# IllyaArtemchuk/Harmonies-Alphazero

Measured on AMD Instinct MI355X. Metric: self-play env-steps/sec + games/sec @4096 boards, 1/2/4/8 GPUs; bit-exact vs CPU, higher is better.
Workload: dtype u64; 1 GPU; config2: 4096 concurrent boards/GPU, reset + rule-driven play to game end (legal mask, step, chance draws, final scoring); one step = 256 hz_play launches of 4096 boards; boards_per_gpu=4096, parallelism=shard1

## Files before the change

### __graft_entry__.py

```python
import os
import subprocess
import sys

ROOT = os.path.dirname(os.path.abspath(__file__))
PKG = os.path.join(ROOT, "harmonies-alphazero_amd")


def _paths():
    for p in (ROOT, PKG):
        if p not in sys.path:
            sys.path.insert(0, p)


def build() -> None:
    jobs = str(min(16, os.cpu_count() or 4))
    subprocess.run(["make", "-s", "-j", jobs, "-C", PKG], check=True)
    subprocess.run(["make", "-s", "-C", os.path.join(ROOT, "oracle")], check=True)
    _paths()
    import hzamd
    import hzamd._native as nat
    missing = [s for s in nat.exported_symbols() if not hasattr(nat.lib(), s)]
    if missing:
        raise RuntimeError(f"libhz.so lacks symbols: {missing}")


def smoke() -> None:
    _paths()
    import numpy as np
    import torch

    import oracle
    from hzamd.env import BatchedEnv
    from hzamd.state import unpack_ref

    n, base = 256, 4242
    env = BatchedEnv(n, seed_base=base, device="cuda:0")
    env.reset()
    games, steps, _ = env.rollout(max_plies=200)
    st = env.export_state().cpu().numpy()
    torch.cuda.synchronize()
    total, finals, plies, _ = oracle.play_rule_games(n, base)
    got = np.stack([unpack_ref(st[:, b]) for b in range(n)])
    assert (got == finals).all(), "final states differ from the oracle"
    assert (steps.cpu().numpy() == plies).all(), "ply counts differ from the oracle"
    assert int(games.sum()) == n
    for _ in range(15):
        games, steps, _ = env.rollout(max_plies=200, reset=True)
    st = env.export_state().cpu().numpy()
    torch.cuda.synchronize()
    env.check_errors()
    _, finals, plies, _ = oracle.play_rule_games(n, base, episode=15)
    got = np.stack([unpack_ref(st[:, b]) for b in range(n)])
    assert (got == finals).all(), "hz_play: final states differ from the oracle"
    assert (steps.cpu().numpy() == plies).all(), "hz_play: ply counts differ from the oracle"
    env.close()
    print(f"smoke ok: {n} boards, {total} env steps bit-exact vs oracle; hz_play episode 15 bit-exact")


if __name__ == "__main__":
    build()
    if len(sys.argv) > 1 and sys.argv[1] == "smoke":
        smoke()
```

### harmonies-alphazero_amd/csrc/hz_env.hip

```cpp
#include <hip/hip_runtime.h>

#include <cstdio>
#include <cstdlib>
#include <cstring>

#include "../../include/hz_abi.h"
#include "hz_device.hpp"
#include "hz_encode.hpp"
#include "hz_host.hpp"

using namespace hz;
using namespace hz_host;

struct P2Draw {
  int32_t *tag;
  int32_t *k;
  uint64_t *q;
  uint64_t *bag;
  int32_t *c;
};
struct P2Mid {
  int32_t *tag;
  uint64_t *st;
  uint64_t *q;
  int32_t *i;
};

#ifndef HZ_P2_NDRAW
#define HZ_P2_NDRAW 5
#endif
#ifndef HZ_P2_NPLAY
#define HZ_P2_NPLAY 5
#endif
constexpr int kP2Draw = HZ_P2_NDRAW;
constexpr int kP2Play = HZ_P2_NPLAY;
constexpr int kP2SDraw = 4;
constexpr int kP2SPlay = kP2SDraw + kP2Draw;
constexpr int kP2Stages = kP2SPlay + kP2Play;
constexpr int kP2Last = kP2Stages - 1;
constexpr int kP2Ring = kP2Play + 1;
constexpr int kP2Stream = kP2Stages;
static_assert(kP2Draw >= 2 && kP2Draw <= 5 && kP2Play >= 2 && kP2Play <= 5, "stage counts");

struct hz_env {
  DevBufs bufs, p2_bufs, ar_bufs;
  int32_t n;
  uint64_t seed_base;
  hipStream_t stream;
  uint64_t *state;
  uint32_t *mt;
  int32_t *pos;
  int32_t *ply;
  int32_t *episode;
  uint64_t *seed;
  int seed_ahead;
  uint32_t *ahead_mt[2];
  int32_t *ahead_tag[2];
  uint64_t *ahead_pile[2];
  int32_t *ahead_cur[2];
  uint32_t *ahead_rule[2];
  int32_t *ep_final[2];
  size_t nrow;
  uint32_t *ring_mt[3];
  int32_t *ring_tag[3];
  uint64_t *ring_pile[3];
  int32_t *ring_cur[3];
  int32_t *ring_k1[3];
  int calls;
  int primed, slot_valid[2];
  int32_t *mt_src;
  int lazy;
  int ar_ahead;
  uint32_t *ar_mt;
  int32_t *ar_tag;
  uint64_t *ar_pile;
  int32_t *ar_cur;
  int32_t *ar_ep[2];
  int ar_calls, ar_primed;
  uint32_t *pw_words;
  int32_t *pw_tag;
  int32_t *pw_ep;
  uint32_t mt_epoch;
  int pipeline;
  int calls2, primed2;
  int p2_cut[kP2Play - 1];
  int p2_dcut[kP2Draw + 1];
  uint32_t *p2_s[kP2Stream];
  int32_t *p2_s_tag[kP2Stream];
  int32_t *p2_s_cur[kP2Stream];
  uint32_t *p2_p1h[2];
  int32_t *p2_p1t[2];
  uint32_t *p2_p2h[2];
  uint32_t *p2_p3h[2];
  P2Draw p2_x[kP2Draw - 1][2];
  P2Draw p2_pl[kP2Ring];
  P2Mid p2_m[kP2Play - 1][2];
  uint32_t *p2_h[kP2Ring];
  int32_t *p2_h_tag[kP2Ring];
  int32_t *p2_ep[2];
  int32_t *wait_err_own;
  int32_t *wait_err;
  int spin_limit;
};

#ifdef HZ_DIAG
__device__ uint64_t *g_stamps;
__device__ int g_role_only = -1;
#define HZ_STAMP(slot)                                                    \
  do {                                                                    \
    __builtin_amdgcn_sched_barrier(0);                                    \
    if (g_stamps) g_stamps[(size_t)b * 16 + (slot)] = __builtin_amdgcn_s_memtime(); \
    __builtin_amdgcn_sched_barrier(0);                                    \
  } while (0)
#ifndef HZ_DIAG_ROLES_ONLY
#define HZ_ACC(slot, t0)                                                  \
  do {                                                                    \
    __builtin_amdgcn_sched_barrier(0);                                    \
    uint64_t _t = __builtin_amdgcn_s_memtime();                           \
    acc##slot += _t - (t0);                                               \
    t0 = _t;                                                              \
    __builtin_amdgcn_sched_barrier(0);                                    \
  } while (0)
#else
#define HZ_ACC(slot, t0) \
  do {                   \
  } while (0)
#endif
#define HZ_PHASE(slot, t0, b)                                                                 \
  do {                                                                                        \
    __builtin_amdgcn_sched_barrier(0);                                                        \
    if (g_stamps) g_stamps[(size_t)(b) * 16 + (slot)] = __builtin_amdgcn_s_memtime() - (t0); \
    __builtin_amdgcn_sched_barrier(0);                                                        \
  } while (0)
#else
#define HZ_STAMP(slot) \
  do {                 \
  } while (0)
#define HZ_PHASE(slot, t0, b) \
  do {                        \
  } while (0)
#define HZ_ACC(slot, t0) \
  do {                   \
  } while (0)
#endif

namespace {

constexpr int kBlock = 64;

inline int grid_for(int n) { return (n + kBlock - 1) / kBlock; }

constexpr int kStageThreads = 256;
constexpr size_t kResetLds = (size_t)kMT * kLdsStride * sizeof(uint32_t);

__device__ __forceinline__ void stage_mt(uint32_t *__restrict__ g, int nb, int tid, uint64_t mask, bool to_lds) {
  uint32_t *lds = hz_lds;
  constexpr int U = 8;
  int total4 = nb * (kMT / 4);
  for (int q0 = 0; q0 < total4; q0 += kStageThreads * U) {
    uint4 v[U];
#pragma unroll
    for (int u = 0; u < U; u++) {
      int q = q0 + u * kStageThreads + tid;
      int o = q * 4, bl = o / kMT, i = o - bl * kMT;
      if (q < total4 && ((mask >> bl) & 1)) {
        if (to_lds) {
          v[u] = reinterpret_cast<const uint4 *>(g)[q];
        } else {
          v[u].x = lds[i * kLdsStride + bl];
          v[u].y = lds[(i + 1) * kLdsStride + bl];
          v[u].z = lds[(i + 2) * kLdsStride + bl];
          v[u].w = lds[(i + 3) * kLdsStride + bl];
        }
      }
    }
#pragma unroll
    for (int u = 0; u < U; u++) {
      int q = q0 + u * kStageThreads + tid;
      int o = q * 4, bl = o / kMT, i = o - bl * kMT;
      if (q < total4 && ((mask >> bl) & 1)) {
        if (to_lds) {
// ... 1036 lines not shown
            steps += done;
            i += done - 1;
            if (phase_of(s.misc) == PH_OVER) games++;
            continue;
          }
        }
        int a;
        HZ_ACC(8, t0);
        if constexpr (Record) {
          uint64_t mk[3];
          int L = legal_mask(s, mk);
          HZ_ACC(9, t0);
          if (traj_state) {
            uint64_t *o = traj_state + (size_t)i * 6 * n + b;
            o[0] = s.pl[0]; o[(size_t)n] = s.pl[1]; o[(size_t)2 * n] = s.pl[2]; o[(size_t)3 * n] = s.pl[3];
            o[(size_t)4 * n] = s.piles; o[(size_t)5 * n] = s.misc;
          }
          if (traj_mask) {
            uint64_t *o = traj_mask + ((size_t)i * n + b) * 3;
            o[0] = mk[0]; o[1] = mk[1]; o[2] = mk[2];
          }
          a = L ? kth_action(mk, rule_pick_k(rkey, g_ply, L)) : -1;
          if (traj_action) traj_action[(size_t)i * n + b] = (int16_t)a;
        } else {
          a = rule_action(s, rule_h32(rkey, g_ply));
          HZ_ACC(9, t0);
        }
        if (a < 0) break;
        HZ_ACC(10, t0);
        bool te = phase_of(s.misc) == PH_P3;
        step_trusted<true>(s, a, draw);
        if (te) HZ_ACC(12, t0);
        else HZ_ACC(11, t0);
        g_ply++;
        steps++;
        if (phase_of(s.misc) == PH_OVER) games++;
      }
    }
#ifdef HZ_DIAG_ROLES_ONLY
    HZ_PHASE(9, role_t0, b);
#endif
    if (score_pending(s.misc)) finish_game(s);
#ifdef HZ_DIAG_ROLES_ONLY
    HZ_PHASE(10, role_t0, b);
#endif
    HZ_ACC(13, t0);
    store_state(st, n, b, s);
    if (lds_used) pos[b] = draw.m.cursor();
    else if (draw.fell) pos[b] = draw.gm.cursor();
    else pos[b] = cur_b[(size_t)draw.d * n];
    mt_src[b] = lds_used ? -1 : src_b;
    ply[b] = g_ply;
    seed[b] = sd;
#if defined(HZ_DIAG) && !defined(HZ_DIAG_ROLES_ONLY)
    if (g_stamps) {
      uint64_t *o = g_stamps + (size_t)b * 16;
      o[8] = acc8; o[9] = acc9; o[10] = acc10; o[11] = acc11; o[12] = acc12; o[13] = acc13;
    }
#endif
    if (games_done) games_done[b] = games;
    if (steps_done) steps_done[b] = steps;
    if (ep_final) ep_final[b] = episode[b];
    uint64_t lm = __ballot(lds_used);
    if (lane == 0) s_lds_mask = lm;
  }
  if (w0 && !act && lane == 0 && actmask == 0) s_lds_mask = 0;
  __syncthreads();
  uint64_t lds_mask = s_lds_mask & actmask;
  if (lds_mask) stage_mt(g, nb, tid, lds_mask, false);
#ifdef HZ_DIAG
  if (g_stamps && threadIdx.x < 64 && act) g_stamps[(size_t)b * 16 + 5] = __builtin_amdgcn_s_memtime() - role_t0;
#endif
}

#ifndef HZ_P2_ST_WT
#define HZ_P2_ST_WT 0
#endif
#ifndef HZ_P2_AUX
#define HZ_P2_AUX 16
#endif
constexpr int kP2Win = 96;
constexpr int kP2WinRows = kP2Win + 24;
#ifndef HZ_P2_DCUT
#if HZ_P2_NDRAW == 5
#define HZ_P2_DCUT 0, 6, 11, 15, 19
#elif HZ_P2_NDRAW == 4
#define HZ_P2_DCUT 0, 7, 13, 18
#endif
#endif
constexpr int kP2DCut[kP2Draw] = {HZ_P2_DCUT};
constexpr int kP2StageDraws = 7;
#ifndef HZ_P2_PCUT
#if HZ_P2_NPLAY == 5
#define HZ_P2_PCUT 16, 32, 48, 64
#elif HZ_P2_NPLAY == 4
#define HZ_P2_PCUT 24, 40, 56
#endif
#endif
constexpr int kP2PCut[kP2Play - 1] = {HZ_P2_PCUT};
enum { kWvP1 = 8, kWvHash = 9, kWvPlay = 10, kWvIdle = 15 };
#ifndef HZ_P2_WAVES
#if HZ_P2_NDRAW == 5 && HZ_P2_NPLAY == 5
#define HZ_P2_WAVES 0, 1, 4, 9, 2, 3, 8, 10
#elif HZ_P2_NDRAW == 5
#define HZ_P2_WAVES 0, 1, 4, 9, 2, 3, 8, 15
#elif HZ_P2_NPLAY == 5
#define HZ_P2_WAVES 0, 1, 8, 9, 2, 3, 10, 15
#else
#define HZ_P2_WAVES 0, 1, 8, 9, 2, 3, 15, 15
#endif
#endif
constexpr int kP2Wave[8] = {HZ_P2_WAVES};
constexpr int p2_wave_count(int code) {
  int c = 0;
  for (int k = 0; k < 8; k++) c += kP2Wave[k] == code;
  return c;
}
constexpr bool p2_waves_ok() {
  for (int d = 0; d < 5; d++)
    if (p2_wave_count(d) != (d < kP2Draw ? 1 : 0)) return false;
  return p2_wave_count(kWvP1) == 1 && p2_wave_count(kWvHash) == 1 && p2_wave_count(kWvPlay) == (kP2Play == 5 ? 1 : 0);
}
static_assert(p2_waves_ok(), "HZ_P2_WAVES: every stage outside the seed and play blocks on exactly one wave");
constexpr int kP2MinPlies = 96;
#ifdef HZ_DIAG
constexpr int kP2Stamps = 48;
#define P2_PHASE(slot, t0)                                                                                       \
  do {                                                                                                           \
    __builtin_amdgcn_sched_barrier(0);                                                                           \
    if (g_stamps && b < a.n) g_stamps[(size_t)b * kP2Stamps + (slot)] = __builtin_amdgcn_s_memtime() - (t0); \
    __builtin_amdgcn_sched_barrier(0);                                                                           \
  } while (0)
#else
#define P2_PHASE(slot, t0) \
  do {                     \
  } while (0)
#endif
static_assert(4 * kP2WinRows * kWinStride * 4 <= (int)kResetLds, "a window per wave of a draw block");

struct P2Args {
  uint64_t *st;
  uint32_t *mt;
  int32_t *pos, *ply, *episode;
  uint64_t *seed;
  int n, max_plies, draws;
  int cut[kP2Play - 1];
  int dcut[kP2Draw + 1];
  uint64_t seed_base;
  long nrow;
  int32_t *games_done, *steps_done, *mt_src;
  const int32_t *ep_in;
  int32_t *ep_out;
  uint32_t *s_mt[kP2Stages];
  int32_t *s_tag[kP2Stages];
  int32_t *s_cur[kP2Stages];
  int s_idx_last;
  uint32_t *p1h_w;
  const uint32_t *p1h_r;
  int32_t *p1t_w;
  const int32_t *p1t_r;
  uint32_t *p2h_w;
  const uint32_t *p2h_r;
  uint32_t *p3h_w;
  const uint32_t *p3h_r;
  P2Draw x_w[kP2Draw - 1], x_r[kP2Draw - 1];
  P2Draw pl_w, pl_r[kP2Play];
  P2Mid m_w[kP2Play - 1], m_r[kP2Play - 1];
  uint32_t *h_w;
  const uint32_t *h_r[kP2Play];
  int32_t *ht_w;
  const int32_t *ht_r[kP2Play];
  int32_t *err;
  int spin;
};

struct PlayDraw2 {
  uint64_t q0, q1, q2, q3;
  int d, nd;
  bool fell;
  MTR gm;
  const int32_t *cur_nd;
  __device__ __forceinline__ uint32_t pop() {
    uint32_t p9 = (uint32_t)q0 & 0x1FFu;
    q0 = (q0 >> 9) | (q1 << 55);
    q1 = (q1 >> 9) | (q2 << 55);
    q2 = (q2 >> 9) | (q3 << 55);
    q3 >>= 9;
    d++;
    return p9;
  }
  __device__ __forceinline__ bool pair_pops() const { return d + 2 <= nd; }
  __device__ __forceinline__ uint32_t draw_one(uint64_t misc) {
    if (d < nd) return pop();
    if (!fell) {
      gm = MTR(gm.w, gm.stride, *cur_nd);
      fell = true;
    }
    uint32_t p9;
    return draw_pile(misc, gm, p9) ? p9 : 0x1FFu;
  }
  __device__ __forceinline__ uint32_t operator()(uint64_t misc) { return take(misc, true); }
  __device__ __forceinline__ uint32_t take(uint64_t misc, bool want) {
    if (__all(!want || d < nd)) {
      uint32_t p9 = want ? (uint32_t)q0 & 0x1FFu : 0x1FFu;
      uint64_t n0 = (q0 >> 9) | (q1 << 55), n1 = (q1 >> 9) | (q2 << 55), n2 = (q2 >> 9) | (q3 << 55);
      q0 = want ? n0 : q0;
      q1 = want ? n1 : q1;
      q2 = want ? n2 : q2;
      q3 = want ? q3 >> 9 : q3;
      d += want ? 1 : 0;
      return p9;
    }
    return want ? draw_one(misc) : 0x1FFu;
  }
  __device__ __forceinline__ void scripted_reset(State &s) {
    s.pl[0] = s.pl[1] = s.pl[2] = s.pl[3] = 0;
    uint64_t open = q0 & ((1ull << 45) - 1);
    s.piles = open | (5ull << 45);
    uint64_t misc = 0x1FF;
#pragma unroll
    for (int t = 0; t < 6; t++) misc = set_bits(misc, 11 + 5 * t, 5, (uint64_t)initial_count(t));
#pragma unroll
    for (int i = 0; i < 5; i++) apply_pile_fast(misc, (uint32_t)(open >> (9 * i)) & 0x1FFu);
    s.misc = misc;
    q0 = (q0 >> 45) | (q1 << 19);
    q1 = (q1 >> 45) | (q2 << 19);
    q2 = (q2 >> 45) | (q3 << 19);
    q3 >>= 45;
    d = 5;
  }
};

template <class Draw>
__device__ __forceinline__ int p2_plies(State &s, Draw &draw, int g, int g_end, uint64_t rkey, const uint32_t *hs,
                                        size_t nr) {
  const int g0 = g;
  auto hash = [&](int ply) -> uint32_t { return hs && ply < kRulePlies ? hs[(size_t)ply * nr] : rule_h32(rkey, ply); };
  const bool all_hs = __all(hs != nullptr);
  uint32_t hn[8];
  int hn_g = -1;
  while (g < g_end) {
    if (phase_of(s.misc) == PH_OVER) break;
    if (__all(g + 8 <= g_end && turn_pair_safe(s))) {
      uint32_t h[8];
      if (__all(hn_g == g)) {
#pragma unroll
        for (int j = 0; j < 8; j++) h[j] = hn[j];
      } else if (all_hs && __all(g + 8 <= kRulePlies)) {
#pragma unroll
        for (int j = 0; j < 8; j++) h[j] = hs[(size_t)(g + j) * nr];
      } else {
#pragma unroll
        for (int j = 0; j < 8; j++) h[j] = hash(g + j);
      }
// ... 371 lines not shown
__device__ __forceinline__ void p2_draw_stage(const P2Args &a, int b0, int lane, int stage, int base) {
  const int b = b0 + lane;
#ifdef HZ_DIAG
  const uint64_t t0 = __builtin_amdgcn_s_memtime();
#endif
  const bool act = b < a.n;
  const size_t nr = (size_t)a.nrow;
  const int d0 = a.dcut[stage], d1 = stage == kP2Draw - 1 ? a.draws : min(a.draws, a.dcut[stage + 1]);
  const int e = act ? a.ep_in[b] + kP2Last - kP2SDraw - stage : 0;
  const uint32_t *slot = a.s_mt[kP2SDraw + stage];
  int32_t *cur = a.s_cur[kP2SDraw + stage] + b;
  const P2Draw &in = a.x_r[stage > 0 ? stage - 1 : 0];
  const P2Draw &out = stage == kP2Draw - 1 ? a.pl_w : a.x_w[stage < kP2Draw - 1 ? stage : 0];
  bool ok = act && a.s_tag[kP2SDraw + stage][b] == e * 8 + 5;
  int k0 = 0, c0 = kMTAhead;
  uint64_t bag = initial_bag(), q[kAheadWords] = {0, 0, 0, 0};
  constexpr int U = kP2Win / 4;
  const int c4 = (lane & 15) * 4;
  uint4 v[U];
  auto win_load = [&](int r0) {
#pragma unroll
    for (int u = 0; u < U; u++) {
      const int r = r0 + 4 * u + (lane >> 4);
      v[u] = p2_ld4(slot + (size_t)r * nr + b0 + c4);
    }
  };
  auto win_store = [&]() {
#pragma unroll
    for (int u = 0; u < U; u++)
      *reinterpret_cast<uint4 *>(hz_lds + base + (4 * u + (lane >> 4)) * kWinStride + c4) = v[u];
  };
  if (stage == 0) win_load(0);
  if (stage > 0 && act) {
    const int itag = in.tag[b];
    k0 = in.k[b];
    c0 = in.c[b];
    bag = in.bag[b];
#pragma unroll
    for (int i = 0; i < kAheadWords; i++) q[i] = in.q[(size_t)i * nr + b];
    ok = ok && itag == e * 8 + stage;
  }
  const bool draws = ok && k0 >= d0 && d0 < d1;
  const int r0 = wave_min_i(draws ? (c0 & 0xFFFF) : kAheadTwist) & ~3;
  if (r0 < kAheadTwist) {
    if (stage > 0) win_load(r0);
    win_store();
  }
  P2_PHASE(28 + stage, t0);
  if (!act) return;
  if (!ok) {
    out.tag[b] = -1;
    return;
  }
  if (stage == 0) cur[0] = kMTAhead;
  int k = k0, cc = c0;
  if (draws) {
    const int lim = min(r0 + kP2Win, kAheadTwist);
    StreamDraw<WinMT> d{WinMT(base - r0 * kWinStride + lane, c0, lim)};
#pragma unroll 1
    for (int i = d0; i < d1; i++) {
      if (d.m.pos >= lim) break;
      const uint32_t p9 = d(bag);
      if (d.m.pos > lim) break;
      apply_pile_fast(bag, p9);
      const int bit = 9 * i, wd = bit >> 6, off = bit & 63;
      const uint64_t lo9 = (uint64_t)p9 << off, hi9 = off > 55 ? (uint64_t)p9 >> (64 - off) : 0ull;
      q[0] |= wd == 0 ? lo9 : 0ull;
      q[1] |= wd == 1 ? lo9 : wd == 0 ? hi9 : 0ull;
      q[2] |= wd == 2 ? lo9 : wd == 1 ? hi9 : 0ull;
      q[3] |= wd == 3 ? lo9 : wd == 2 ? hi9 : 0ull;
      cc = d.m.cursor();
      p2_st(&cur[(size_t)(i + 1) * nr], cc);
      k = i + 1;
    }
  }
  p2_st(&out.k[b], k);
  p2_st(&out.c[b], cc);
  p2_st(&out.bag[b], bag);
#pragma unroll
  for (int i = 0; i < kAheadWords; i++) p2_st(&out.q[(size_t)i * nr + b], q[i]);
  p2_st(&out.tag[b], e * 8 + stage + 1);
}

__device__ __forceinline__ void p2_hashes(const P2Args &a, int b) {
  const size_t nr = (size_t)a.nrow;
  const int e = a.ep_in[b] + kP2Last - (kP2SPlay - 1);
  const uint64_t rk = rule_key(episode_seed(a.seed_base, b, e));
#pragma unroll 1
  for (int j = 0; j < kRulePlies; j++) p2_st(&a.h_w[(size_t)j * nr + b], rule_h32(rk, j));
  a.ht_w[b] = e;
}

__device__ __forceinline__ void p2_draw(const P2Args &a, int blk, int code) {
  const int tid = threadIdx.x, lane = tid & 63, w = tid >> 6;
  const int b0 = blk * kBlock;
  if (code < kP2Draw) {
    p2_draw_stage(a, b0, lane, code, w * kP2WinRows * kWinStride);
  } else if (code == kWvP1 && b0 + lane < a.n) {
    p2_p1(a, b0 + lane);
  } else if (code == kWvHash && b0 + lane < a.n) {
    p2_hashes(a, b0 + lane);
  }
}

__device__ __forceinline__ void p2_mid_put(const P2Mid &m, size_t nr, int b, const State &s, const PlayDraw2 &d, int g,
                                           int e) {
#pragma unroll
  for (int k = 0; k < 4; k++) p2_st(&m.st[(size_t)k * nr + b], s.pl[k]);
  p2_st(&m.st[4 * nr + b], s.piles);
  p2_st(&m.st[5 * nr + b], s.misc);
  p2_st(&m.q[b], d.q0);
  p2_st(&m.q[nr + b], d.q1);
  p2_st(&m.q[2 * nr + b], d.q2);
  p2_st(&m.q[3 * nr + b], d.q3);
  p2_st(&m.i[b], d.d);
  p2_st(&m.i[nr + b], g);
  p2_st(&m.i[2 * nr + b], d.fell ? d.gm.cursor() : -1);
  p2_st(&m.tag[b], e);
}
__device__ __forceinline__ PlayDraw2 p2_mid_get(const P2Mid &m, size_t nr, int b, State &s, int &g, int nd,
                                               uint32_t *slot, const int32_t *cur) {
#pragma unroll
  for (int k = 0; k < 4; k++) s.pl[k] = m.st[(size_t)k * nr + b];
  s.piles = m.st[4 * nr + b];
  s.misc = m.st[5 * nr + b];
  const int d = m.i[b], fc = m.i[2 * nr + b];
  g = m.i[nr + b];
  return PlayDraw2{m.q[b], m.q[nr + b], m.q[2 * nr + b], m.q[3 * nr + b], d, nd, fc >= 0,
                   MTR(slot, (int)nr, fc >= 0 ? fc : 0), cur + (size_t)nd * nr};
}

__device__ __forceinline__ void p2_play(const P2Args &a, int blk, int st, bool in_block) {
  __shared__ uint64_t s_lds_mask;
  const int tid = threadIdx.x, lane = tid & 63, w = tid >> 6;
  const int b0 = blk * kBlock, b = b0 + lane;
  const bool act = b < a.n;
  const uint64_t actmask = __ballot(act);
  const int nb = a.n - b0 < kBlock ? a.n - b0 : kBlock;
  const size_t nr = (size_t)a.nrow;
#ifdef HZ_DIAG
  const uint64_t t0 = __builtin_amdgcn_s_memtime();
#endif
  const bool last = st == kP2Play - 1;
  bool lds_used = false;
  if (act) {
    const int e = last ? a.episode[b] : a.ep_in[b] + kP2Play - 1 - st;
    const P2Draw &pl = a.pl_r[st];
    const uint32_t *hsrc = a.h_r[st];
    const int32_t *htag = a.ht_r[st];
    uint32_t *slot = a.s_mt[kP2SPlay + st] + b;
    const int32_t *cur = a.s_cur[kP2SPlay + st] + b;
    const int g_end = last ? a.max_plies : min(a.cut[st < kP2Play - 1 ? st : 0], a.max_plies);
    const uint64_t sd = episode_seed(a.seed_base, b, e), rk = rule_key(sd);
    const int ptag = pl.tag[b], nd = pl.k[b];
    const int mtag = st > 0 ? a.m_r[st - 1].tag[b] : e;
    const uint32_t *hs = htag[b] == e ? hsrc + b : nullptr;
    State s;
    int g = 0;
    PlayDraw2 draw = st == 0 ? PlayDraw2{pl.q[b], pl.q[nr + b], pl.q[2 * nr + b], pl.q[3 * nr + b], 0, nd, false,
                                         MTR(slot, (int)nr, 0), cur + (size_t)nd * nr}
                             : p2_mid_get(a.m_r[st - 1], nr, b, s, g, nd, slot, cur);
    const bool prep = ptag == e * 8 + kP2Draw && mtag == e;
    if (prep) {
      if (st == 0) {
        if (__all(nd >= 5)) draw.scripted_reset(s);
        else reset_state(s, draw);
      }
      P2_PHASE(16 + 2 * st, t0);
      g += p2_plies(s, draw, g, g_end, rk, hs, nr);
      P2_PHASE(17 + 2 * st, t0);
    }
    if (!last) {
      const P2Mid &mo = a.m_w[st < kP2Play - 1 ? st : 0];
      if (prep) p2_mid_put(mo, nr, b, s, draw, g, e);
      else mo.tag[b] = -1;
    } else {
      int cursor, src;
      if (prep) {
        cursor = draw.fell ? draw.gm.cursor() : cur[(size_t)draw.d * nr];
        src = 2 + a.s_idx_last;
      } else {
        mt_seed(hz_lds + lane, kLdsStride, sd);
        PlayDraw fb{LdsMT(lane, kMTSeeded), false, false, 0, 0, 0, 0, 0, 0, MT(nullptr, 0), nullptr};
        reset_state(s, fb);
        g = p2_plies(s, fb, 0, a.max_plies, rk, nullptr, nr);
        cursor = fb.m.cursor();
        src = -1;
        lds_used = true;
      }
      a.episode[b] = e + 1;
      if (score_pending(s.misc)) finish_game(s);
      P2_PHASE(27, t0);
      store_state(a.st, a.n, b, s);
      a.pos[b] = cursor;
      a.mt_src[b] = src;
      a.ply[b] = g;
      a.seed[b] = sd;
      a.ep_out[b] = e + 1;
      if (a.games_done) a.games_done[b] = phase_of(s.misc) == PH_OVER ? 1 : 0;
      if (a.steps_done) a.steps_done[b] = g;
    }
#ifdef HZ_DIAG
    if (g_stamps && in_block) g_stamps[(size_t)b * kP2Stamps + w] = __builtin_amdgcn_s_memtime() - t0;
#endif
  }
  if (!in_block) return;
  if (w == 0) {
    const uint64_t lm = __ballot(lds_used);
    if (lane == 0) s_lds_mask = lm;
  }
  __syncthreads();
  const uint64_t lds_mask = s_lds_mask & actmask;
  if (lds_mask) stage_mt(a.mt + (size_t)b0 * kMT, nb, tid, lds_mask, false);
}

__global__ void __launch_bounds__(kStageThreads) __attribute__((amdgpu_waves_per_eu(1, 1))) k_play2(P2Args a, int nblk) {
  const int blk = (int)blockIdx.x;
  const int role = blk / nblk;
  const int rb = blk - role * nblk;
  const int wv = __builtin_amdgcn_readfirstlane((int)(threadIdx.x >> 6));
  const int code = role == 1 || role == 2 ? kP2Wave[4 * (role - 1) + wv] : kWvIdle;
  const int st = role == 0 ? kP2Play - 1 - wv : code == kWvPlay ? 0 : -1;
#ifdef HZ_DIAG
  if (g_role_only >= 0 && g_role_only != role) return;
  const uint64_t t0 = __builtin_amdgcn_s_memtime(), r0 = __builtin_amdgcn_s_memrealtime();
#endif
  if (st >= 0) p2_play(a, rb, st, role == 0);
  else if (role == 3) p2_seed(a, rb);
  else if (role != 0) p2_draw(a, rb, code);
#ifdef HZ_DIAG
  {
    const int w = threadIdx.x >> 6, bb = rb * kBlock + (threadIdx.x & 63);
    const bool idle = (role == 1 || role == 2) && code == kWvIdle;
    if (g_stamps && role > 0 && !idle && bb < a.n) g_stamps[(size_t)bb * kP2Stamps + 4 * role + w] = __builtin_amdgcn_s_memtime() - t0;
    if (g_stamps && bb < a.n && (threadIdx.x & 63) < 4) {
      const int k = threadIdx.x & 63;
      const uint64_t v = k == 0 ? r0 : k == 1 ? __builtin_amdgcn_s_memrealtime() : k == 2 ? t0 : __builtin_amdgcn_s_memtime();
      g_stamps[(size_t)(rb * kBlock + 16 * role + 4 * w + k) * kP2Stamps + 40] = v;
      if (k == 0)
        g_stamps[(size_t)(rb * kBlock + 16 * role + 4 * w) * kP2Stamps + 41] =
            (uint64_t)__builtin_amdgcn_s_getreg((31 << 11) | 4) | ((uint64_t)__builtin_amdgcn_s_getreg((15 << 11) | 20) << 32);
    }
  }
#endif
}
// ... 71 lines not shown
  int b = blockIdx.x * blockDim.x + threadIdx.x;
  if (b >= n) return;
  MT m(mt + (size_t)b * kMT, pos[b]);
  m.normalize();
  pos[b] = m.cursor();
  if (index) index[b] = m.pos;
}

__global__ void __launch_bounds__(kBlock) k_mt_import(int32_t *__restrict__ pos, int n,
                                                      const int32_t *__restrict__ index) {
  int b = blockIdx.x * blockDim.x + threadIdx.x;
  if (b >= n) return;
  pos[b] = index[b] | (kMT << 16);
}

}

__global__ void __launch_bounds__(64) k_mt_materialize(uint32_t *__restrict__ mt, const uint32_t *__restrict__ a0,
                                                      const uint32_t *__restrict__ a1, int32_t *__restrict__ mt_src,
                                                      int n) {
  const int b = blockIdx.x, lane = threadIdx.x;
  const int src = mt_src[b];
  if (src < 0 || src > 1) return;
  const uint32_t *from = (src ? a1 : a0) + (size_t)b * kMT;
  uint32_t *to = mt + (size_t)b * kMT;
  uint32_t v[(kMT + 63) / 64];
#pragma unroll
  for (int k = 0; k < (kMT + 63) / 64; k++) v[k] = lane + 64 * k < kMT ? from[lane + 64 * k] : 0u;
#pragma unroll
  for (int k = 0; k < (kMT + 63) / 64; k++)
    if (lane + 64 * k < kMT) to[lane + 64 * k] = v[k];
  if (lane == 0) mt_src[b] = -1;
}

__global__ void __launch_bounds__(64) k_mt_materialize_ar(uint32_t *__restrict__ mt, const uint32_t *__restrict__ ar_mt,
                                                         int32_t *__restrict__ mt_src, int n) {
  const int b = blockIdx.x, lane = threadIdx.x;
  const int src = mt_src[b];
  if (src < kArSrc || src >= kArSrc + kArSlots) return;
  const uint32_t *from = ar_mt + ((size_t)(src - kArSrc) * n + b) * kMT;
  uint32_t *to = mt + (size_t)b * kMT;
  uint32_t v[(kMT + 63) / 64];
#pragma unroll
  for (int k = 0; k < (kMT + 63) / 64; k++) v[k] = lane + 64 * k < kMT ? from[lane + 64 * k] : 0u;
#pragma unroll
  for (int k = 0; k < (kMT + 63) / 64; k++)
    if (lane + 64 * k < kMT) to[lane + 64 * k] = v[k];
  if (lane == 0) mt_src[b] = -1;
}

static PlyWin ply_win(hz_env *e) {
  return PlyWin{e->pw_words, e->pw_tag, e->pw_ep, (long)e->nrow, (int32_t)e->mt_epoch};
}

static int materialize(hz_env *e) {
  if (!e->lazy) return 0;
  streams_touched(e);
  if (e->ar_mt)
    hipLaunchKernelGGL(k_mt_materialize_ar, dim3(e->n), dim3(64), 0, e->stream, e->mt, e->ar_mt, e->mt_src, e->n);
  hipLaunchKernelGGL(k_mt_materialize, dim3(e->n), dim3(64), 0, e->stream, e->mt, e->ahead_mt[0], e->ahead_mt[1],
                     e->mt_src, e->n);
  if (e->p2_s[0]) {
    P2Slots sl;
    for (int k = 0; k < kP2Stream; k++) sl.s[k] = e->p2_s[k];
    hipLaunchKernelGGL(k_mt_materialize2, dim3(e->n), dim3(64), 0, e->stream, e->mt, sl, e->mt_src,
                       (long)e->nrow);
  }
  e->lazy = 0;
  return launch_err();
}

static_assert(sizeof(((hz_env *)0)->p2_s) / sizeof(uint32_t *) == kP2Stream, "slot ring");

static int p2_clear_tags(hz_env *e) {
  const size_t bytes = e->nrow * sizeof(int32_t);
  auto c = [&](int32_t *t) { return hipMemsetAsync(t, 0xff, bytes, e->stream) != hipSuccess; };
  for (int k = 0; k < kP2Stream; k++)
    if (c(e->p2_s_tag[k])) return 1;
  for (int k = 0; k < 2; k++)
    if (c(e->p2_p1t[k])) return 1;
  for (int k = 0; k < kP2Draw - 1; k++)
    if (c(e->p2_x[k][0].tag) || c(e->p2_x[k][1].tag)) return 1;
  for (int k = 0; k < kP2Ring; k++)
    if (c(e->p2_pl[k].tag) || c(e->p2_h_tag[k])) return 1;
  for (int k = 0; k < kP2Play - 1; k++)
    if (c(e->p2_m[k][0].tag) || c(e->p2_m[k][1].tag)) return 1;
  return 0;
}

static int alloc_p2(hz_env *e) {
  if (e->p2_s[0]) return 0;
  const size_t nr = e->nrow;
  DevBufs &o = e->p2_bufs;
  for (int k = 0; k < kP2Stream; k++) {
    o.get(e->p2_s[k], nr * kMT * 4);
    o.get(e->p2_s_tag[k], nr * 4);
    o.get(e->p2_s_cur[k], (kAheadDraws + 1) * nr * 4);
  }
  auto md = [&](P2Draw &d) {
    o.get(d.tag, nr * 4);
    o.get(d.k, nr * 4);
    o.get(d.q, kAheadWords * nr * 8);
    o.get(d.bag, nr * 8);
    o.get(d.c, nr * 4);
  };
  for (int k = 0; k < kP2Draw - 1; k++) md(e->p2_x[k][0]), md(e->p2_x[k][1]);
  for (int k = 0; k < kP2Ring; k++) {
    md(e->p2_pl[k]);
    o.get(e->p2_h[k], kRulePlies * nr * 4);
    o.get(e->p2_h_tag[k], nr * 4);
  }
  for (int k = 0; k < kP2Play - 1; k++)
    for (int j = 0; j < 2; j++) {
      P2Mid &mm = e->p2_m[k][j];
      o.get(mm.tag, nr * 4);
      o.get(mm.st, 6 * nr * 8);
      o.get(mm.q, 4 * nr * 8);
      o.get(mm.i, 3 * nr * 4);
    }
  for (int k = 0; k < 2; k++) {
    o.get(e->p2_p1h[k], nr * 4);
    o.get(e->p2_p1t[k], nr * 4);
    o.get(e->p2_p2h[k], 4 * nr * 4);
    o.get(e->p2_p3h[k], 4 * nr * 4);
    o.get(e->p2_ep[k], nr * 4);
  }
  if (!o.ok || p2_clear_tags(e)) {
    o.release();
    return 1;
  }
  e->primed2 = 0;
  return 0;
}

static int launch_play2(hz_env *e, int32_t max_plies, int32_t *games_done, int32_t *steps_done) {
  streams_touched(e);
  if (alloc_p2(e)) return 1;
  const int c = e->calls2, r = c & 1, w = r ^ 1;
  if (!e->primed2) {
    if (hipMemcpyAsync(e->p2_ep[w], e->episode, (size_t)e->n * sizeof(int32_t), hipMemcpyDeviceToDevice,
                       e->stream))
      return 1;
    e->primed2 = 1;
  }
  P2Args a{};
  a.st = e->state;
  a.mt = e->mt;
  a.pos = e->pos;
  a.ply = e->ply;
  a.episode = e->episode;
  a.seed = e->seed;
  a.n = e->n;
  a.max_plies = max_plies;
  a.draws = e->seed_ahead;
  a.err = e->wait_err;
  a.spin = e->spin_limit;
  for (int k = 0; k < kP2Play - 1; k++) a.cut[k] = e->p2_cut[k];
  for (int k = 0; k <= kP2Draw; k++) a.dcut[k] = e->p2_dcut[k];
  a.seed_base = e->seed_base;
  a.nrow = (long)e->nrow;
  a.games_done = games_done;
  a.steps_done = steps_done;
  a.mt_src = e->mt_src;
  a.ep_in = e->p2_ep[w];
  a.ep_out = e->p2_ep[r];
  auto sl = [c](int s) { return ((c - s) % kP2Stream + kP2Stream) % kP2Stream; };
  for (int s = 1; s < kP2Stages; s++) {
    a.s_mt[s] = e->p2_s[sl(s)];
    a.s_tag[s] = e->p2_s_tag[sl(s)];
    a.s_cur[s] = e->p2_s_cur[sl(s)];
  }
  a.s_idx_last = sl(kP2Last);
  a.p1h_w = e->p2_p1h[r];
  a.p1h_r = e->p2_p1h[w];
  a.p1t_w = e->p2_p1t[r];
  a.p1t_r = e->p2_p1t[w];
  a.p2h_w = e->p2_p2h[r];
  a.p2h_r = e->p2_p2h[w];
  a.p3h_w = e->p2_p3h[r];
  a.p3h_r = e->p2_p3h[w];
  for (int k = 0; k < kP2Draw - 1; k++) {
    a.x_w[k] = e->p2_x[k][r];
    a.x_r[k] = e->p2_x[k][w];
  }
  a.pl_w = e->p2_pl[c % kP2Ring];
  a.h_w = e->p2_h[c % kP2Ring];
  a.ht_w = e->p2_h_tag[c % kP2Ring];
  for (int st = 0; st < kP2Play; st++) {
    const int k = (c + kP2Ring - 1 - st) % kP2Ring;
    a.pl_r[st] = e->p2_pl[k];
    a.h_r[st] = e->p2_h[k];
    a.ht_r[st] = e->p2_h_tag[k];
  }
  for (int st = 0; st < kP2Play - 1; st++) {
    a.m_w[st] = e->p2_m[st][r];
    a.m_r[st] = e->p2_m[st][w];
  }
  const int nblk = grid_for(e->n);
  hipLaunchKernelGGL(k_play2, dim3(4 * nblk), dim3(kStageThreads), kResetLds, e->stream, a, nblk);
  if (int err = launch_err()) return err;
  e->lazy = 1;
  e->calls2 = (c + 1) % (kP2Stream * kP2Ring * 2);
  e->primed = 0;
  e->ar_primed = 0;
  return 0;
}

extern "C" {

hz_env *hz_env_create(int32_t n_boards, uint64_t seed_base, void *stream) {
  if (n_boards <= 0) return nullptr;
  if (install_comp_table()) return nullptr;
  if (lds_opt_in<k_reset>(kResetLds) || lds_opt_in<k_rollout<false, false>>(kResetLds) ||
      lds_opt_in<k_rollout<false, true>>(kResetLds) || lds_opt_in<k_rollout<true, false>>(kResetLds) ||
      lds_opt_in<k_rollout<true, true>>(kResetLds) || lds_opt_in<k_play2>(kResetLds))
    return nullptr;
  hz_env *e = new (std::nothrow) hz_env();
  if (!e) return nullptr;
  e->n = n_boards;
  e->seed_base = seed_base;
  e->stream = (hipStream_t)stream;
  const size_t n = (size_t)n_boards, nr = (n + kBlock - 1) / kBlock * kBlock, i32 = sizeof(int32_t);
  e->nrow = nr;
  DevBufs &o = e->bufs;
  o.get(e->state, n * 6 * sizeof(uint64_t), 0);
  o.get(e->mt, n * 624 * sizeof(uint32_t));
  o.get(e->pos, n * i32, 0);
  o.get(e->ply, n * i32, 0);
  o.get(e->episode, n * i32, 0);
  o.get(e->seed, n * sizeof(uint64_t), 0);
  o.get(e->mt_src, n * i32, 0xff);
  for (int k = 0; k < 2; k++) {
    o.get(e->ahead_mt[k], n * kMT * sizeof(uint32_t));
    o.get(e->ahead_tag[k], n * i32, 0xff);
    o.get(e->ahead_pile[k], n * kAheadWords * sizeof(uint64_t));
    o.get(e->ahead_cur[k], n * (kAheadDraws + 1) * i32);
    o.get(e->ahead_rule[k], nr * kRulePlies * sizeof(uint32_t));
    o.get(e->ep_final[k], n * i32);
  }
  for (int k = 0; k < kRing; k++) {
    o.get(e->ring_mt[k], nr * kMT * sizeof(uint32_t));
    o.get(e->ring_tag[k], nr * i32, 0xff);
    o.get(e->ring_pile[k], nr * 3 * sizeof(uint64_t));
    o.get(e->ring_cur[k], nr * (kD1Draws + 1) * i32);
    o.get(e->ring_k1[k], nr * i32);
  }
  o.get(e->pw_words, nr * kPlyWin * sizeof(uint32_t));
  o.get(e->pw_tag, nr * i32, 0xff);
  o.get(e->pw_ep, nr * i32, 0);
  o.get(e->wait_err_own, i32, 0);
  e->seed_ahead = kAheadDraws;
  e->ar_ahead = env_pick("HZ_AR_AHEAD", 0, 1);
  e->pipeline = env_pick("HZ_PIPELINE", 1, 2);
  for (int k = 0; k < kP2Play - 1; k++) e->p2_cut[k] = kP2PCut[k];
  if constexpr (kP2Play == 4) env_cuts("HZ_P2_CUTS", e->p2_cut);
  else if constexpr (kP2Play == 5) env_cuts_n("HZ_P2_CUTS5", e->p2_cut, kP2Play - 1, 4, 1 << 20);
  for (int k = 0; k < kP2Draw; k++) e->p2_dcut[k] = kP2DCut[k];
  e->p2_dcut[kP2Draw] = kAheadDraws;
  if constexpr (kP2Draw == 5) {
    int dc[kP2Draw + 1];
    for (int k = 0; k <= kP2Draw; k++) dc[k] = e->p2_dcut[k];
    if (env_cuts_n("HZ_P2_DCUTS", dc + 1, kP2Draw - 1, 1, kAheadDraws - 1) &&
        cuts_gaps_within(dc, kP2Draw + 1, kP2StageDraws))
      for (int k = 0; k <= kP2Draw; k++) e->p2_dcut[k] = dc[k];
  }
  e->mt_epoch = 1;
  e->wait_err = e->wait_err_own;
  e->spin_limit = kSpinLimitDefault;
  if (!o.ok || hipDeviceSynchronize() != hipSuccess) {
    hz_env_destroy(e);
    return nullptr;
  }
  return e;
}

void hz_env_destroy(hz_env *e) {
  if (!e) return;
  e->p2_bufs.release();
  e->ar_bufs.release();
  e->bufs.release();
  delete e;
}

int32_t hz_env_size(const hz_env *e) { return e ? e->n : -1; }

int hz_env_set_error_word(hz_env *e, int32_t *word) {
  if (!e) return -1;
  e->wait_err = word ? word : e->wait_err_own;
  return 0;
}

int hz_env_set_spin_limit(hz_env *e, int32_t limit) {
  if (!e || limit < 0) return -1;
  e->spin_limit = limit ? limit : kSpinLimitDefault;
  return 0;
}

int hz_env_set_pipeline(hz_env *e, int32_t pipeline) {
  if (!e || (pipeline != 1 && pipeline != 2)) return -1;
  e->pipeline = pipeline;
  e->primed = 0;
  e->primed2 = 0;
  return 0;
}

int hz_env_set_auto_ahead(hz_env *e, int32_t on) {
  if (!e) return -1;
  e->ar_ahead = on ? 1 : 0;
  e->ar_primed = 0;
  return 0;
}

int hz_env_set_stream(hz_env *e, void *stream) {
  if (!e) return -1;
  e->stream = (hipStream_t)stream;
  return 0;
}

uint64_t *hz_env_state_ptr(hz_env *e) { return e ? e->state : nullptr; }
uint32_t *hz_env_mt_ptr(hz_env *e) {
  if (!e || materialize(e)) return nullptr;
  streams_touched(e);
  return e->mt;
}
int32_t *hz_env_mt_pos_ptr(hz_env *e) {
  if (!e) return nullptr;
  streams_touched(e);
  return e->pos;
}
int32_t *hz_env_ply_ptr(hz_env *e) { return e ? e->ply : nullptr; }
uint64_t *hz_env_seed_ptr(hz_env *e) { return e ? e->seed : nullptr; }

int hz_env_set_seed_ahead(hz_env *e, int32_t draws) {
  if (!e || draws < 0) return -1;
  e->seed_ahead = draws > kAheadDraws ? kAheadDraws : draws;
  e->primed = 0;
  e->primed2 = 0;
  if (e->p2_s[0] && p2_clear_tags(e)) return 1;
  for (int k = 0; k < kRing; k++)
    if (hipMemsetAsync(e->ring_tag[k], 0xff, e->nrow * sizeof(int32_t), e->stream)) return 1;
  return 0;
}

int hz_reset(hz_env *e, const uint8_t *sel, const uint64_t *seeds) {
  if (!e) return -1;
  streams_touched(e);
  if (int err = materialize(e)) return err;
  e->primed = 0;
// ... 247 lines not shown
```

### harmonies-alphazero_amd/csrc/hz_host.hpp

```cpp
#pragma once

#include <atomic>
#include <cstddef>
#include <cstdint>
#include <cstdio>
#include <cstdlib>
#include <new>
#include <vector>

namespace hz_host {

inline int env_int(const char *name, int dflt) {
  const char *e = getenv(name);
  return e ? atoi(e) : dflt;
}

inline int env_pick(const char *name, int special, int otherwise) {
  return env_int(name, otherwise) == special ? special : otherwise;
}

inline int env_clamped(const char *name, int dflt, int lo, int hi) {
  const int v = env_int(name, dflt);
  return v < lo ? lo : v > hi ? hi : v;
}

inline void env_cuts(const char *name, int cut[3]) {
  const char *e = getenv(name);
  int c[3];
  if (e && sscanf(e, "%d,%d,%d", &c[0], &c[1], &c[2]) == 3 && c[0] > 0 && c[1] > c[0] && c[2] > c[1] &&
      c[0] % 4 == 0 && c[1] % 4 == 0 && c[2] % 4 == 0)
    for (int k = 0; k < 3; k++) cut[k] = c[k];
}

inline bool env_cuts_n(const char *name, int *cut, int n, int step, int hi) {
  const char *e = getenv(name);
  if (!e || n < 1 || n > 8 || step < 1) return false;
  int c[8];
  for (int k = 0; k < n; k++) {
    if (*e < '0' || *e > '9') return false;
    long v = 0;
    for (; *e >= '0' && *e <= '9'; e++)
      if ((v = v * 10 + (*e - '0')) > hi) return false;
    if (v < step || v % step || (k && v <= c[k - 1])) return false;
    c[k] = (int)v;
    if (*e++ != (k + 1 < n ? ',' : '\0')) return false;
  }
  for (int k = 0; k < n; k++) cut[k] = c[k];
  return true;
}

inline bool cuts_gaps_within(const int *cut, int n, int max_gap) {
  for (int k = 0; k + 1 < n; k++)
    if (cut[k + 1] - cut[k] > max_gap) return false;
  return true;
}

struct Setting {
  static constexpr int64_t kUnread = INT64_MIN;
  const char *name;
  int32_t dflt;
  std::atomic<int64_t> v{kUnread};
  int32_t get() {
    int64_t x = v.load(std::memory_order_relaxed);
    if (x == kUnread) {
      int64_t expect = kUnread;
      v.compare_exchange_strong(expect, (int64_t)env_int(name, dflt));
      x = v.load(std::memory_order_relaxed);
    }
    return (int32_t)x;
  }
  void set(int32_t x) { v.store(x, std::memory_order_relaxed); }
};

template <class Dev>
struct DevBufsT {
  struct Held {
    void *p;
    void *slot;
    void (*clear)(void *slot);
  };
  std::vector<Held> held;
  bool ok = true;

  template <class T>
  bool get(T *&p, size_t bytes) {
    if (!ok) return false;
    void *raw = nullptr;
    if (!Dev::alloc(&raw, bytes)) return ok = false;
    p = static_cast<T *>(raw);
    held.push_back(Held{raw, &p, [](void *s) { *static_cast<T **>(s) = nullptr; }});
    return true;
  }
  template <class T>
  bool get(T *&p, size_t bytes, int byte) {
    return get(p, bytes) && (ok = Dev::fill(p, byte, bytes));
  }
  template <class T>
  bool get(T *&p, size_t bytes, int byte, void *stream) {
    return get(p, bytes) && (ok = Dev::fill_async(p, byte, bytes, stream));
  }
  void release() {
    for (const Held &h : held) {
      Dev::free(h.p);
      h.clear(h.slot);
    }
    held.clear();
    ok = true;
  }
};

template <class Env>
inline void streams_touched(Env *e) {
  e->mt_epoch++;
}

}

#ifdef __HIPCC__
#include <hip/hip_runtime.h>

namespace hz_host {

struct HipDev {
  static bool alloc(void **p, size_t bytes) { return hipMalloc(p, bytes) == hipSuccess; }
  static bool fill(void *p, int byte, size_t bytes) { return hipMemset(p, byte, bytes) == hipSuccess; }
  static bool fill_async(void *p, int byte, size_t bytes, void *stream) {
    return hipMemsetAsync(p, byte, bytes, (hipStream_t)stream) == hipSuccess;
  }
  static void free(void *p) { (void)hipFree(p); }
};
using DevBufs = DevBufsT<HipDev>;

inline int launch_err() {
  hipError_t e = hipGetLastError();
  return e == hipSuccess ? 0 : (int)e;
}
// ... 18 lines not shown
```

Before: 22.77 billion env-steps/s.

## Fold rule-hash computation into play stages and add sixth draw stage

Removes the dedicated hash wave that precomputed per-ply rule hashes into a ring buffer with tags. Each play stage now computes the hashes for its own ply range inline into a per-stage buffer, and the freed wave slot becomes a sixth draw stage with new draw cut points. The goal is to rebalance work across the waves of the pipelined kernel and drop the ring and tag bookkeeping. In exchange, play stages take on extra hash arithmetic, and the host cut-parsing helper is generalized.

```diff
diff --git a/__graft_entry__.py b/__graft_entry__.py
--- a/__graft_entry__.py
+++ b/__graft_entry__.py
@@ -44,17 +44,17 @@
     assert (got == finals).all(), "final states differ from the oracle"
     assert (steps.cpu().numpy() == plies).all(), "ply counts differ from the oracle"
     assert int(games.sum()) == n
-    for _ in range(15):
+    for _ in range(16):
         games, steps, _ = env.rollout(max_plies=200, reset=True)
     st = env.export_state().cpu().numpy()
     torch.cuda.synchronize()
     env.check_errors()
-    _, finals, plies, _ = oracle.play_rule_games(n, base, episode=15)
+    _, finals, plies, _ = oracle.play_rule_games(n, base, episode=16)
     got = np.stack([unpack_ref(st[:, b]) for b in range(n)])
     assert (got == finals).all(), "hz_play: final states differ from the oracle"
     assert (steps.cpu().numpy() == plies).all(), "hz_play: ply counts differ from the oracle"
     env.close()
-    print(f"smoke ok: {n} boards, {total} env steps bit-exact vs oracle; hz_play episode 15 bit-exact")
+    print(f"smoke ok: {n} boards, {total} env steps bit-exact vs oracle; hz_play episode 16 bit-exact")
 
 
 if __name__ == "__main__":
diff --git a/harmonies-alphazero_amd/csrc/hz_env.hip b/harmonies-alphazero_amd/csrc/hz_env.hip
--- a/harmonies-alphazero_amd/csrc/hz_env.hip
+++ b/harmonies-alphazero_amd/csrc/hz_env.hip
@@ -27,7 +27,7 @@
 };
 
 #ifndef HZ_P2_NDRAW
-#define HZ_P2_NDRAW 5
+#define HZ_P2_NDRAW 6
 #endif
 #ifndef HZ_P2_NPLAY
 #define HZ_P2_NPLAY 5
@@ -40,7 +40,7 @@
 constexpr int kP2Last = kP2Stages - 1;
 constexpr int kP2Ring = kP2Play + 1;
 constexpr int kP2Stream = kP2Stages;
-static_assert(kP2Draw >= 2 && kP2Draw <= 5 && kP2Play >= 2 && kP2Play <= 5, "stage counts");
+static_assert(kP2Draw >= 2 && kP2Draw <= 6 && kP2Play >= 2 && kP2Play <= 5, "stage counts");
 
 struct hz_env {
   DevBufs bufs, p2_bufs, ar_bufs;
@@ -95,8 +95,7 @@
   P2Draw p2_x[kP2Draw - 1][2];
   P2Draw p2_pl[kP2Ring];
   P2Mid p2_m[kP2Play - 1][2];
-  uint32_t *p2_h[kP2Ring];
-  int32_t *p2_h_tag[kP2Ring];
+  uint32_t *p2_hs[kP2Play];
   int32_t *p2_ep[2];
   int32_t *wait_err_own;
   int32_t *wait_err;
@@ -1299,7 +1298,9 @@
 constexpr int kP2Win = 96;
 constexpr int kP2WinRows = kP2Win + 24;
 #ifndef HZ_P2_DCUT
-#if HZ_P2_NDRAW == 5
+#if HZ_P2_NDRAW == 6
+#define HZ_P2_DCUT 0, 5, 9, 13, 17, 21
+#elif HZ_P2_NDRAW == 5
 #define HZ_P2_DCUT 0, 6, 11, 15, 19
 #elif HZ_P2_NDRAW == 4
 #define HZ_P2_DCUT 0, 7, 13, 18
@@ -1315,16 +1316,20 @@
 #endif
 #endif
 constexpr int kP2PCut[kP2Play - 1] = {HZ_P2_PCUT};
-enum { kWvP1 = 8, kWvHash = 9, kWvPlay = 10, kWvIdle = 15 };
+enum { kWvP1 = 8, kWvPlay = 10, kWvIdle = 15 };
 #ifndef HZ_P2_WAVES
-#if HZ_P2_NDRAW == 5 && HZ_P2_NPLAY == 5
-#define HZ_P2_WAVES 0, 1, 4, 9, 2, 3, 8, 10
+#if HZ_P2_NDRAW == 6 && HZ_P2_NPLAY == 5
+#define HZ_P2_WAVES 0, 1, 4, 5, 2, 3, 8, 10
+#elif HZ_P2_NDRAW == 6
+#define HZ_P2_WAVES 0, 1, 4, 5, 2, 3, 8, 15
+#elif HZ_P2_NDRAW == 5 && HZ_P2_NPLAY == 5
+#define HZ_P2_WAVES 0, 1, 4, 15, 2, 3, 8, 10
 #elif HZ_P2_NDRAW == 5
-#define HZ_P2_WAVES 0, 1, 4, 9, 2, 3, 8, 15
+#define HZ_P2_WAVES 0, 1, 4, 15, 2, 3, 8, 15
 #elif HZ_P2_NPLAY == 5
-#define HZ_P2_WAVES 0, 1, 8, 9, 2, 3, 10, 15
+#define HZ_P2_WAVES 0, 1, 8, 15, 2, 3, 10, 15
 #else
-#define HZ_P2_WAVES 0, 1, 8, 9, 2, 3, 15, 15
+#define HZ_P2_WAVES 0, 1, 8, 15, 2, 3, 15, 15
 #endif
 #endif
 constexpr int kP2Wave[8] = {HZ_P2_WAVES};
@@ -1334,9 +1339,9 @@
   return c;
 }
 constexpr bool p2_waves_ok() {
-  for (int d = 0; d < 5; d++)
+  for (int d = 0; d < 6; d++)
     if (p2_wave_count(d) != (d < kP2Draw ? 1 : 0)) return false;
-  return p2_wave_count(kWvP1) == 1 && p2_wave_count(kWvHash) == 1 && p2_wave_count(kWvPlay) == (kP2Play == 5 ? 1 : 0);
+  return p2_wave_count(kWvP1) == 1 && p2_wave_count(kWvPlay) == (kP2Play == 5 ? 1 : 0);
 }
 static_assert(p2_waves_ok(), "HZ_P2_WAVES: every stage outside the seed and play blocks on exactly one wave");
 constexpr int kP2MinPlies = 96;
@@ -1383,10 +1388,7 @@
   P2Draw x_w[kP2Draw - 1], x_r[kP2Draw - 1];
   P2Draw pl_w, pl_r[kP2Play];
   P2Mid m_w[kP2Play - 1], m_r[kP2Play - 1];
-  uint32_t *h_w;
-  const uint32_t *h_r[kP2Play];
-  int32_t *ht_w;
-  const int32_t *ht_r[kP2Play];
+  uint32_t *hs[kP2Play];
   int32_t *err;
   int spin;
 };
@@ -1924,15 +1926,6 @@
   p2_st(&out.tag[b], e * 8 + stage + 1);
 }
 
-__device__ __forceinline__ void p2_hashes(const P2Args &a, int b) {
-  const size_t nr = (size_t)a.nrow;
-  const int e = a.ep_in[b] + kP2Last - (kP2SPlay - 1);
-  const uint64_t rk = rule_key(episode_seed(a.seed_base, b, e));
-#pragma unroll 1
-  for (int j = 0; j < kRulePlies; j++) p2_st(&a.h_w[(size_t)j * nr + b], rule_h32(rk, j));
-  a.ht_w[b] = e;
-}
-
 __device__ __forceinline__ void p2_draw(const P2Args &a, int blk, int code) {
   const int tid = threadIdx.x, lane = tid & 63, w = tid >> 6;
   const int b0 = blk * kBlock;
@@ -1940,8 +1933,6 @@
     p2_draw_stage(a, b0, lane, code, w * kP2WinRows * kWinStride);
   } else if (code == kWvP1 && b0 + lane < a.n) {
     p2_p1(a, b0 + lane);
-  } else if (code == kWvHash && b0 + lane < a.n) {
-    p2_hashes(a, b0 + lane);
   }
 }
 
@@ -1988,21 +1979,24 @@
   if (act) {
     const int e = last ? a.episode[b] : a.ep_in[b] + kP2Play - 1 - st;
     const P2Draw &pl = a.pl_r[st];
-    const uint32_t *hsrc = a.h_r[st];
-    const int32_t *htag = a.ht_r[st];
+    uint32_t *hsw = a.hs[st] + b;
     uint32_t *slot = a.s_mt[kP2SPlay + st] + b;
     const int32_t *cur = a.s_cur[kP2SPlay + st] + b;
     const int g_end = last ? a.max_plies : min(a.cut[st < kP2Play - 1 ? st : 0], a.max_plies);
     const uint64_t sd = episode_seed(a.seed_base, b, e), rk = rule_key(sd);
     const int ptag = pl.tag[b], nd = pl.k[b];
     const int mtag = st > 0 ? a.m_r[st - 1].tag[b] : e;
-    const uint32_t *hs = htag[b] == e ? hsrc + b : nullptr;
     State s;
     int g = 0;
     PlayDraw2 draw = st == 0 ? PlayDraw2{pl.q[b], pl.q[nr + b], pl.q[2 * nr + b], pl.q[3 * nr + b], 0, nd, false,
                                          MTR(slot, (int)nr, 0), cur + (size_t)nd * nr}
                              : p2_mid_get(a.m_r[st - 1], nr, b, s, g, nd, slot, cur);
+    const int h_lo = st > 0 ? a.cut[st - 1] : 0;
+    const int h_hi = min(last ? kRulePlies : a.cut[st < kP2Play - 1 ? st : 0], kRulePlies);
+#pragma unroll 1
+    for (int j = h_lo; j < h_hi; j++) hsw[(size_t)j * nr] = rule_h32(rk, j);
     const bool prep = ptag == e * 8 + kP2Draw && mtag == e;
+    const uint32_t *hs = g >= h_lo ? hsw : nullptr;
     if (prep) {
       if (st == 0) {
         if (__all(nd >= 5)) draw.scripted_reset(s);
@@ -2240,7 +2234,7 @@
   for (int k = 0; k < kP2Draw - 1; k++)
     if (c(e->p2_x[k][0].tag) || c(e->p2_x[k][1].tag)) return 1;
   for (int k = 0; k < kP2Ring; k++)
-    if (c(e->p2_pl[k].tag) || c(e->p2_h_tag[k])) return 1;
+    if (c(e->p2_pl[k].tag)) return 1;
   for (int k = 0; k < kP2Play - 1; k++)
     if (c(e->p2_m[k][0].tag) || c(e->p2_m[k][1].tag)) return 1;
   return 0;
@@ -2263,11 +2257,8 @@
     o.get(d.c, nr * 4);
   };
   for (int k = 0; k < kP2Draw - 1; k++) md(e->p2_x[k][0]), md(e->p2_x[k][1]);
-  for (int k = 0; k < kP2Ring; k++) {
-    md(e->p2_pl[k]);
-    o.get(e->p2_h[k], kRulePlies * nr * 4);
-    o.get(e->p2_h_tag[k], nr * 4);
-  }
+  for (int k = 0; k < kP2Ring; k++) md(e->p2_pl[k]);
+  for (int k = 0; k < kP2Play; k++) o.get(e->p2_hs[k], kRulePlies * nr * 4);
   for (int k = 0; k < kP2Play - 1; k++)
     for (int j = 0; j < 2; j++) {
       P2Mid &mm = e->p2_m[k][j];
@@ -2342,13 +2333,10 @@
     a.x_r[k] = e->p2_x[k][w];
   }
   a.pl_w = e->p2_pl[c % kP2Ring];
-  a.h_w = e->p2_h[c % kP2Ring];
-  a.ht_w = e->p2_h_tag[c % kP2Ring];
   for (int st = 0; st < kP2Play; st++) {
     const int k = (c + kP2Ring - 1 - st) % kP2Ring;
     a.pl_r[st] = e->p2_pl[k];
-    a.h_r[st] = e->p2_h[k];
-    a.ht_r[st] = e->p2_h_tag[k];
+    a.hs[st] = e->p2_hs[st];
   }
   for (int st = 0; st < kP2Play - 1; st++) {
     a.m_w[st] = e->p2_m[st][r];
@@ -2415,13 +2403,7 @@
   else if constexpr (kP2Play == 5) env_cuts_n("HZ_P2_CUTS5", e->p2_cut, kP2Play - 1, 4, 1 << 20);
   for (int k = 0; k < kP2Draw; k++) e->p2_dcut[k] = kP2DCut[k];
   e->p2_dcut[kP2Draw] = kAheadDraws;
-  if constexpr (kP2Draw == 5) {
-    int dc[kP2Draw + 1];
-    for (int k = 0; k <= kP2Draw; k++) dc[k] = e->p2_dcut[k];
-    if (env_cuts_n("HZ_P2_DCUTS", dc + 1, kP2Draw - 1, 1, kAheadDraws - 1) &&
-        cuts_gaps_within(dc, kP2Draw + 1, kP2StageDraws))
-      for (int k = 0; k <= kP2Draw; k++) e->p2_dcut[k] = dc[k];
-  }
+  if constexpr (kP2Draw == 6) env_draw_cuts("HZ_P2_DCUTS", e->p2_dcut, kP2Draw, kAheadDraws, kP2StageDraws);
   e->mt_epoch = 1;
   e->wait_err = e->wait_err_own;
   e->spin_limit = kSpinLimitDefault;
diff --git a/harmonies-alphazero_amd/csrc/hz_host.hpp b/harmonies-alphazero_amd/csrc/hz_host.hpp
--- a/harmonies-alphazero_amd/csrc/hz_host.hpp
+++ b/harmonies-alphazero_amd/csrc/hz_host.hpp
@@ -52,6 +52,20 @@
 inline bool cuts_gaps_within(const int *cut, int n, int max_gap) {
   for (int k = 0; k + 1 < n; k++)
     if (cut[k + 1] - cut[k] > max_gap) return false;
+  return true;
+}
+
+inline bool env_draw_cuts(const char *name, int *dcut, int stages, int total, int max_gap) {
+  if (stages < 3 || stages > 8) return false;
+  int dc[9] = {0};
+  int set = stages;
+  if (!env_cuts_n(name, dc + 1, stages - 1, 1, total - 1)) {
+    if (!env_cuts_n(name, dc + 1, stages - 2, 1, total - 1)) return false;
+    set = stages - 1;
+  }
+  for (int k = set; k <= stages; k++) dc[k] = total;
+  if (!cuts_gaps_within(dc, stages + 1, max_gap)) return false;
+  for (int k = 0; k <= stages; k++) dcut[k] = dc[k];
   return true;
 }
 
```

Result: no change. 22.76 billion env-steps/s, median of 2 (-0.0%).
